# intel-aero/aero-optical-flow

Measured on AMD Instinct MI355X. Metric: frame-pairs/s (640x480, 8x8 SAD, +-4 search), higher is better.
Workload: dtype u8

## Files before the change

### aero-optical-flow_amd/csrc/aof_batch.cpp

```cpp
#include <cerrno>

#include "aof_ctx.hpp"

using namespace aof;

namespace {

struct Timed {
    aof_ctx *ctx; int id; hipStream_t s; bool on; int slot;
    Timed(aof_ctx *c, int k, hipStream_t st)
        : ctx(c), id(k), s(st), on(c->prof.on && !c->capturing && ((c->prof.mask >> k) & 1u)),
          slot((int)(c->prof.count[k] % AOF_PROFILE_RING))
    {
        if (on) (void)hipEventRecord(ctx->prof.ev[id][slot][0], s);
    }
    ~Timed() { if (on) { (void)hipEventRecord(ctx->prof.ev[id][slot][1], s); ctx->prof.count[id]++; } }
};

struct BatchView {
    const uint8_t *prev, *cur;
    int64_t stride;
    uint32_t *sums;
    uint8_t *l1_prev, *l1_cur;
    aof_block *blocks1; uint8_t *subdirs1; aof_flow *flows1; uint8_t *hist1;
    aof_block *blocks0; uint8_t *subdirs0; aof_flow *flows; uint8_t *hist0;
    uint32_t *hints;
};

enum SearchKind { SK_TILE16, SK_LANE8_GROUP, SK_LANE8, SK_GENERIC };
enum CoarseKind { COARSE_NONE, COARSE_FUSED, COARSE_K1 };

struct LevelPlan {
    SearchKind kind;
    bool refine;
    SearchArgs a;
    FlowTail tail;
};

struct BatchPlan {
    bool small;
    SmallArgs sm;
    CoarseKind coarse;
    bool k1_pass;
    bool sequence;
    CoarseArgs fused;
    PyramidArgs k1;
    LevelPlan level[2];
};

BatchView batch_view(const aof_ctx *ctx, const aof_ws_layout &L, const uint8_t *d_prev, const uint8_t *d_cur,
                     int64_t pair_stride, aof_block *d_blocks, uint8_t *d_subdirs, aof_flow *d_flows, void *d_workspace)
{
    const aof_params &p = ctx->params;
    BatchView v;
    uint8_t *ws = static_cast<uint8_t *>(d_workspace);
    const bool two = p.pyramid_levels == 2, eq = p.mean_subtract != 0;
    v.prev = d_prev; v.cur = d_cur; v.stride = pair_stride;
    v.sums = eq ? reinterpret_cast<uint32_t *>(ws + L.sums) : nullptr;
    v.l1_prev = two ? ws + L.l1_prev : nullptr;
    v.l1_cur = two ? ws + L.l1_cur : nullptr;
    v.blocks1 = reinterpret_cast<aof_block *>(ws + L.l1_blocks);
    v.subdirs1 = p.subpixel ? ws + L.l1_subdirs : nullptr;
    v.flows1 = reinterpret_cast<aof_flow *>(ws + L.l1_flows);
    v.hist1 = ws + L.l1_hist;
    v.blocks0 = d_blocks ? d_blocks : reinterpret_cast<aof_block *>(ws + L.l0_blocks);
    v.subdirs0 = nullptr;
    if (p.subpixel) v.subdirs0 = d_subdirs ? d_subdirs : ws + L.l0_subdirs;
    v.flows = d_flows;
    v.hist0 = ws + L.l0_hist;
    v.hints = p.tile == 16 ? reinterpret_cast<uint32_t *>(ws + L.hints) : nullptr;
    return v;
}

SearchArgs search_args(const aof_ctx *ctx, int level, const uint8_t *prev, const uint8_t *cur, int64_t stride,
                       aof_block *blocks, uint8_t *subdirs, const aof_flow *pred, const uint32_t *sums, int64_t n)
{
    const aof_params &p = ctx->params;
    SearchArgs a;
    a.prev = prev; a.cur = cur; a.pair_stride = stride;
    a.w = p.width >> level; a.h = p.height >> level;
    a.tile = p.tile; a.search = p.search;
    a.grid = level ? ctx->g1 : ctx->g0;
    a.feature_threshold = p.feature_threshold;
    a.value_threshold = value_threshold_u16(p);
    a.subpixel = p.subpixel;
    a.blocks = blocks; a.subdirs = p.subpixel ? subdirs : nullptr;
    a.pred = pred; a.sums = sums; a.level = level; a.n_pairs = n;
    a.hist_range = level_range(p, level);
    a.prune = ctx->search_mode;
    a.hints = nullptr;
    return a;
}

// ... 6 lines not shown
    if (a->prune && tile16_supported(x)) {
        a->prune = 0;
        return SK_TILE16;
    }
    if (lane8_supported(*a)) return lane8_group(*a) > 0 ? SK_LANE8_GROUP : SK_LANE8;
    return SK_GENERIC;
}

constexpr int64_t kSmallMaxPairs = 128;

FlowTail flow_tail(const aof_ctx *ctx, int level, aof_flow *flows, const aof_flow *pred)
{
    const aof_params &p = ctx->params;
    FlowTail t;
    t.nblocks = (level ? ctx->g1 : ctx->g0).blocks(); t.range = level_range(p, level);
    t.hist_filter = p.hist_filter; t.min_valid = p.min_valid;
    t.flows = flows; t.pred = pred; t.emit_predictor = level ? 1 : 0;
    return t;
}

LevelPlan plan_level(const aof_ctx *ctx, SearchArgs a, const FlowTail &tail)
{
    const SearchKind kind = search_kind(ctx, &a);
    return {kind, kind == SK_TILE16 && a.subpixel && !tile16_refines(a), a, tail};
}

BatchPlan plan_batch(const aof_ctx *ctx, const BatchView &v, int64_t n, bool k1_ready)
{
    const aof_params &p = ctx->params;
    const bool two = p.pyramid_levels == 2, eq = p.mean_subtract != 0;
    const int64_t frame = (int64_t)p.width * p.height, l1_frame = (int64_t)(p.width / 2) * (p.height / 2);
    BatchPlan P = {};
    const SmallArgs &sm = P.sm = {search_args(ctx, 0, v.prev, v.cur, v.stride, v.blocks0, v.subdirs0, nullptr, v.sums, n),
                                  search_args(ctx, 1, v.l1_prev, v.l1_cur, l1_frame, v.blocks1, v.subdirs1, nullptr, v.sums, n),
                                  flow_tail(ctx, 0, v.flows, two ? v.flows1 : nullptr), flow_tail(ctx, 1, v.flows1, nullptr),
                                  v.sums, two ? 2 : 1};
    SearchArgs a0 = sm.l0;
    a0.pred = sm.t0.pred;
    a0.hints = v.hints;
    P.level[0] = plan_level(ctx, a0, sm.t0);

    P.small = !ctx->force_generic && !ctx->split_coarse && n <= kSmallMaxPairs && P.level[0].kind == SK_LANE8_GROUP &&
              (!two || plan_level(ctx, sm.l1, sm.t1).kind == SK_LANE8_GROUP) && flow_small_supported(sm);
    if (P.small || (!two && !eq)) return P;

    CoarseArgs &c = P.fused;
    c.prev = v.prev; c.cur = v.cur; c.pair_stride = v.stride;
    c.w = p.width; c.h = p.height; c.tile = p.tile; c.search = p.search; c.subpixel = p.subpixel;
    c.grid = ctx->g1;
    c.feature_threshold = p.feature_threshold;
    c.value_threshold = value_threshold_u16(p);
    c.sums = v.sums; c.blocks = v.blocks1; c.tail = sm.t1; c.n_pairs = n;
    c.first_generation = ctx->cus; c.stagger_groups = 0; c.stagger_ticks = 0;
    if (two && !ctx->force_generic && !ctx->split_coarse && coarse_fused_supported(P.fused)) {
        P.coarse = COARSE_FUSED;
        return P;
    }
    P.coarse = COARSE_K1;
    const bool seq = P.sequence = v.cur - v.prev == frame && v.stride == frame && v.l1_cur >= v.l1_prev;
    P.k1 = {v.prev, seq ? nullptr : v.cur, v.stride, p.width, p.height, v.l1_prev, seq ? nullptr : v.l1_cur, v.sums,
            seq ? n + 1 : n, seq ? 1 : 0};
    P.k1_pass = !(P.sequence && k1_ready);
    if (two) {
// ... 24 lines not shown
        }
        if (arrived * 4 >= st.expected && seen) {
            st.stats.paying_pct = (int32_t)(paying * 100u / seen);
            st.belief = paying * 100u >= seen * kPayingPct ? 1 : 0;
            st.stats.belief = st.belief;
            st.stats.reports_read++;
        }
    }
    if (st.belief != 0) return true;
    if (++st.since_probe >= kProbeEvery) {
        st.since_probe = 0;
        return true;
    }
    return false;
}

enum Capture { CAPTURE_NONE, CAPTURE_ACTIVE, CAPTURE_UNKNOWN };

struct Lane8Launch {
    int prune;
    bool cols;
    bool fused;
    PruneReport rep;
};

VoteMem vote_mem(const aof_ctx *ctx) { return {ctx->votes.mem, kVoteStride, ctx->h_fault, ctx->votes.deadline_ticks}; }

Lane8Launch choose_lane8(aof_ctx *ctx, const SearchArgs &a, Capture cap)
{
    Lane8Launch l = {a.prune, false, false, {nullptr, 0, 1, 0}};
    if (l.prune && ctx->search_mode == AOF_SEARCH_ADAPTIVE) {
        AdaptiveSearch &st = ctx->adapt;
        if (!adaptive_lane8_prunes(st, a)) {
            l.prune = 0;
            st.stats.exhaustive_launches++;
        } else {
            l.prune = st.belief == 1 ? 1 : 2;
            if (++st.launch_no % 0x10000u == 0) st.launch_no++;
            l.rep.slots = st.slots;
            l.rep.launch_no = st.launch_no & 0xFFFFu;
            st.stats.pruned_launches++;
        }
    }
    SearchArgs x = a;
    x.prune = l.prune;
    l.cols = l.prune && lane8_cols_supported(x);
    const VoteMem vm = vote_mem(ctx);
    const bool fits = l.cols ? lane8_cols_votes_supported(x, vm, ctx->votes.pairs)
                             : (!l.prune && lane8_votes_supported(x, vm, ctx->votes.pairs));
    l.fused = fits && !ctx->votes.separate && (cap == CAPTURE_ACTIVE || (cap == CAPTURE_NONE && !ctx->votes.captured));
    return l;
}

int launch_lane8(aof_ctx *ctx, SearchArgs a, const FlowTail &tail, hipStream_t s, bool *reduced)
{
    hipStreamCaptureStatus status = hipStreamCaptureStatusNone;
    const Capture cap = hipStreamIsCapturing(s, &status) != hipSuccess ? CAPTURE_UNKNOWN
                        : status == hipStreamCaptureStatusNone         ? CAPTURE_NONE
                                                                       : CAPTURE_ACTIVE;
    Lane8Launch l = choose_lane8(ctx, a, cap);
    a.prune = l.prune;
    const bool eager = cap == CAPTURE_NONE;
    if (l.fused && eager && ctx->votes.used && ctx->votes.stream != s && hipStreamWaitEvent(s, ctx->votes.done, 0) != hipSuccess)
        return fail(ctx, -EIO, "cannot order the launch behind the context's previous one");
    const VoteMem vm = vote_mem(ctx);
    const FlowTail *t = l.fused ? &tail : nullptr;
    const VoteMem *m = l.fused ? &vm : nullptr;
    PruneReport *rep = l.prune ? &l.rep : nullptr;
    int rc = l.cols ? launch_search_lane8_cols(a, s, rep, t, m) : launch_search_lane8(a, s, t, m, rep);
    if (!rc && l.fused && eager) {
        rc = (int)hipEventRecord(ctx->votes.done, s);
        ctx->votes.stream = s;
        ctx->votes.used = true;
    } else if (!rc && l.fused) {
        ctx->votes.captured = true;
    }
    *reduced = l.fused;
    if (rep && l.rep.slots) ctx->adapt.expected = l.rep.expected;
    return rc;
}


int enqueue_level(aof_ctx *ctx, const LevelPlan &l, uint8_t *hist, int kid_search, int kid_reduce, hipStream_t s)
{
    bool reduced = l.kind == SK_LANE8_GROUP;
    {
        Timed t(ctx, kid_search, s);
        int rc;
        switch (l.kind) {
        case SK_TILE16:
            rc = launch_search_tile16(l.a, s);
            if (!rc && l.refine) rc = launch_refine(l.a, s);
            break;
        case SK_LANE8_GROUP:
            rc = launch_flow_lane8(l.a, l.tail, s);
            break;
        case SK_LANE8:
            rc = launch_lane8(ctx, l.a, l.tail, s, &reduced);
            if (rc < 0) return rc;
            break;
        default:
            rc = launch_search_generic(l.a, s);
        }
        if (rc) return fail(ctx, -EIO, "search launch: %s", hipGetErrorString((hipError_t)rc));
    }
    if (reduced) return 0;
    const ReduceArgs r = {l.a.blocks, l.a.subdirs, value_threshold_u16(ctx->params), l.tail, l.a.n_pairs, nullptr, 0,
                          reinterpret_cast<uint32_t *>(hist)};
    Timed t(ctx, kid_reduce, s);
    const int rc = launch_reduce(r, s);
    if (rc) return fail(ctx, -EIO, "reduce launch: %s", hipGetErrorString((hipError_t)rc));
    return 0;
}

int flow_batch(aof_ctx *ctx, const uint8_t *d_prev, const uint8_t *d_cur, int64_t pair_stride, int64_t n_pairs,
               aof_block *d_blocks, uint8_t *d_subdirs, aof_flow *d_flows, void *d_workspace, size_t workspace_bytes,
               void *stream, bool k1_ready)
{
    if (!ctx) return -EINVAL;
    if (n_pairs < 0 || (n_pairs > 0 && (!d_prev || !d_cur || !d_flows)))
        return fail(ctx, -EINVAL, "null frame or flow pointer");
    if (int sticky = sticky_error(ctx)) return sticky;
    if (n_pairs == 0) return 0;
    const aof_params &p = ctx->params;
    if (pair_stride < (int64_t)p.width * p.height && n_pairs > 1)
        return fail(ctx, -EINVAL, "pair_stride smaller than a frame");
    aof_ws_layout L;
    int rc = aof_workspace_layout(&p, n_pairs, &L);
    if (rc) return fail(ctx, rc, "bad workspace layout");
    if (!d_workspace || workspace_bytes < L.total_bytes)
        return fail(ctx, -ENOSPC, "workspace %zu B < required %zu B", workspace_bytes, L.total_bytes);
// ... 85 lines not shown
```

### aero-optical-flow_amd/csrc/aof_cols8_kernels.hpp

```cpp
#pragma once

#include <type_traits>

#include "aof_cols8_plan.hpp"
#include "aof_device.hpp"
#include "aof_internal.hpp"
#include "aof_lane8.hpp"
#include "aof_reduce.hpp"
#include "aof_refine.hpp"

namespace aof {

namespace {

template <bool SUBPIXEL, bool VOTE>
__device__ __forceinline__ void cols_walk(const SearchArgs &a, const ColsPlan &plan, const PruneReport &report, const VoteMem *votes)
{
    const uint32_t wg = blockIdx.x;
    const uint32_t unit0 = wg * blockDim.x + threadIdx.x;
    const bool in_tail = (uint32_t)__builtin_amdgcn_readfirstlane((int)unit0) >= plan.head_units;
    const ColsSegments sg = in_tail ? plan.tail : plan.head;
    const uint32_t unit = in_tail ? unit0 - plan.head_units : unit0;
    const uint32_t pair = (in_tail ? plan.head_pairs : 0u) + (uint32_t)__builtin_amdgcn_readfirstlane((int)fast_div(unit, sg.div_units));
    if (pair >= (uint32_t)a.n_pairs) return;
    const uint32_t local = unit - (pair - (in_tail ? plan.head_pairs : 0u)) * sg.units_per_pair;
    const uint32_t seg = fast_div(local, plan.div_nx), bx = local - __umul24(seg, (uint32_t)a.grid.nx);
    const bool live = local < (uint32_t)(sg.segs * a.grid.nx);
    const int by0 = (int)seg * sg.len;
    const int W = a.w;
    constexpr int m = SUBPIXEL ? 1 : 0;

    const uint64_t span = a.n_pairs > 1 ? (uint64_t)(a.n_pairs - pair) * (uint64_t)a.pair_stride : (uint64_t)a.w * (uint64_t)a.h;
    const uint32_t records = span > 0xFFFFFFFFull ? 0xFFFFFFFFu : (uint32_t)span;
    const int64_t base = (int64_t)pair * a.pair_stride;
    const __amdgpu_buffer_rsrc_t rs_prev = __builtin_amdgcn_make_buffer_rsrc(const_cast<uint8_t *>(a.prev) + base, 0, records, kRawBuffer);
    const __amdgpu_buffer_rsrc_t rs_cur = __builtin_amdgcn_make_buffer_rsrc(const_cast<uint8_t *>(a.cur) + base, 0, records, kRawBuffer);
    typedef const __attribute__((address_space(4))) uint32_t *const_u32;
    int px = 0, py = 0, delta = 0;
    if (a.pred) {
        const uint32_t w3 = ((const_u32)(a.pred + pair))[3];
// ... 31 lines not shown
    };
    uint4 win[16];
    {
        const int wy0 = a.grid.y0 + by0 * a.grid.step_y + py - 4;
        const uint32_t off_cur = (uint32_t)(__mul24(wy0, W) + wx0);
        if (mis != 0) {
            shifted_rows(off_cur, win);
        } else if (live) {
#pragma unroll
            for (int s = 0; s < 8; s++) {
                const u32x4 v = __builtin_amdgcn_raw_buffer_load_b128(rs_cur, off_cur, s * W, 0);
                win[s] = make_uint4(v.x, v.y, v.z, v.w);
            }
        }
        if (live && delta != 0) {
#pragma unroll
            for (int s = 0; s < 8; s++) win[s] = sat_add_u8x16(win[s], delta);
        }
    }
    int start_row = a.pred ? 4 : -1, prune_pays = a.prune == 2 ? 0 : 1;
    int seen = 0, paying = 0;
    std::conditional_t<VOTE && !SUBPIXEL, WalkVotes, NoWalkVotes> pending;
    pending.init();
    for (int step = 0; step < sg.len; step++) {
        const int by = by0 + step;
        const bool act = live && by < a.grid.ny;
        if (__ballot(act) == 0) break;
        const int j = a.grid.y0 + by * a.grid.step_y;
        const int wy0 = j + py - 4;
        const bool inside = act && column_inside && wy0 - m >= 0 && wy0 + 16 + m <= a.h;
        const uint32_t off_prev = (uint32_t)(__mul24(j, W) + i);
        const uint32_t off_cur8 = (uint32_t)(__mul24(wy0 + 8, W) + wx0);
        uint32_t ref[8][2];
        if (act) {
#pragma unroll
            for (int r = 0; r < 8; r++) {
                const u32x2 v = __builtin_amdgcn_raw_buffer_load_b64(rs_prev, off_prev, r * W, 2);
                ref[r][0] = v.x; ref[r][1] = v.y;
            }
            if (mis == 0) {
#pragma unroll
                for (int s = 8; s < 16; s++) {
                    const u32x4 v = __builtin_amdgcn_raw_buffer_load_b128(rs_cur, off_cur8, (s - 8) * W, 0);
                    win[s] = make_uint4(v.x, v.y, v.z, v.w);
                }
            }
// ... 46 lines not shown
                    if (!have_ring && rec.sad != 0) {
                        const uint32_t ring = off_cur8 + (uint32_t)((dyi - 9) * W + (dxi - 1));
                        uint32_t rows[10][3];
                        load_ring(rs_cur, ring, W, records, rows);
                        for_rows<-1, 8>([&](auto yc) {
                            constexpr int Y = decltype(yc)::value;
                            uint32_t d[3] = {rows[Y + 1][0], rows[Y + 1][1], rows[Y + 1][2]};
                            if (delta != 0) {
#pragma unroll
                                for (int q = 0; q < 3; q++) d[q] = sat_add_u8x4(d[q], delta);
                            }
                            st.template row<Y>(d, ref);
                        });
                    }
                    subdir = st.direction(rec.sad);
                }
            }
        }
        if (act) {
            const uint32_t slot = (uint32_t)(by * a.grid.nx) + bx;
            slots[slot] = __builtin_bit_cast(uint32_t, rec);
            if constexpr (SUBPIXEL) dirs[slot] = (uint8_t)subdir;
        }
        if constexpr (VOTE) {
            const bool ok = act && (uint32_t)rec.sad < (uint32_t)a.value_threshold;
            int hx = 0, hy = 0;
            if constexpr (SUBPIXEL) {
                hx = (subdir == 0 || subdir == 1 || subdir == 7) ? 1 : ((subdir == 3 || subdir == 4 || subdir == 5) ? -1 : 0);
                hy = (subdir == 1 || subdir == 2 || subdir == 3) ? 1 : ((subdir == 5 || subdir == 6 || subdir == 7) ? -1 : 0);
            }
            const int centre = 2 * a.hist_range + 1;
            if constexpr (SUBPIXEL) vote_and_arrive(*votes, a.hist_range, pair, act, ok, 2 * rec.dx + hx + centre, 2 * rec.dy + hy + centre);
            else pending.step(*votes, a.hist_range, pair, act, ok, 2 * rec.dx + hx + centre, 2 * rec.dy + hy + centre);
        }
#pragma unroll
        for (int s = 0; s < 8; s++) win[s] = win[s + 8];
    }
    if constexpr (VOTE) pending.flush(*votes, a.hist_range, pair);
    if (report.slots && threadIdx.x == 0 && wg % report.stride == 0)
        __hip_atomic_store(report.slots + wg / report.stride, (report.launch_no << 16) | ((uint32_t)paying << 8) | (uint32_t)seen,
                           __ATOMIC_RELAXED, __HIP_MEMORY_SCOPE_SYSTEM);
}

template <bool SUBPIXEL>
__global__ __launch_bounds__(kColsThreads, 4) void k_search_lane8_cols(SearchArgs a, ColsPlan plan, PruneReport report)
{
    cols_walk<SUBPIXEL, false>(a, plan, report, nullptr);
}

template <bool SUBPIXEL>
__global__ __launch_bounds__(kColsThreads, 4) void k_flow_lane8_cols(SearchArgs a, ColsPlan plan, PruneReport report, ColsVotes cv)
{
    if (blockIdx.x >= cv.search_wgs) {
        const uint32_t pair = (blockIdx.x - cv.search_wgs) * (blockDim.x >> 6) + (threadIdx.x >> 6);
        if (pair < (uint32_t)a.n_pairs) await_votes_and_finalise(cv.votes, cv.tail, pair);
        return;
    }
    cols_walk<SUBPIXEL, true>(a, plan, report, &cv.votes);
}

}

}
```

### aero-optical-flow_amd/csrc/aof_cols8_plan.hpp

```cpp
#pragma once

#include <cstdint>

#include "aof_internal.hpp"

namespace aof {

struct ColsSegments {
    int32_t segs, len;
    uint32_t units_per_pair;
    FastDiv div_units;
};
struct ColsPlan {
    ColsSegments head, tail;
    uint32_t head_pairs, head_units;
    FastDiv div_nx;
    uint32_t aligned;
};
struct ColsVotes {
    uint32_t search_wgs;
    FlowTail tail;
    VoteMem votes;
};


constexpr int kColsThreads = 256;
constexpr int kColsMaxRows = 8, kColsMinRows = 2;
constexpr int64_t kColsWavesWanted = 3072;
constexpr int64_t kWaveSlots = 4096;

}
```

### aero-optical-flow_amd/csrc/aof_internal.hpp

```cpp
#pragma once

#include <cstddef>
#include <cstdint>

#include "aof.h"

#if defined(__HIPCC__)
#define AOF_HD __host__ __device__
#else
#define AOF_HD
#endif

namespace aof {

struct FastDiv {
    uint32_t mul, shift;
};
inline FastDiv fastdiv_make(uint32_t d)
{
    FastDiv f = {0u, 0u};
    if (d == 0) return f;
    uint32_t l = 0;
    while ((1ull << l) < d) l++;
    f.mul = (uint32_t)(((1ull << 32) * ((1ull << l) - d)) / d + 1);
// ... 48 lines not shown
    int32_t value_threshold;
    int32_t subpixel;
    aof_block *blocks;
    uint8_t *subdirs;
    const aof_flow *pred;
    const uint32_t *sums;
    int32_t level;
    int64_t n_pairs;
    int32_t hist_range;
    int32_t prune;
    uint32_t *hints;
    FastDiv div_nb, div_nx;
};

struct ReduceArgs {
    const aof_block *blocks;
    const uint8_t *subdirs;
    int32_t value_threshold;
    FlowTail tail;
    int64_t n_pairs;
    const uint32_t *parts;
    int32_t nstrips;
    uint32_t *chunk_parts;
};

struct CoarseArgs {
    const uint8_t *prev, *cur;
    int64_t pair_stride;
    int32_t w, h;
    int32_t tile, search, subpixel;
    Grid grid;
    int32_t feature_threshold;
    int32_t value_threshold;
    uint32_t *sums;
    aof_block *blocks;
    FlowTail tail;
    int64_t n_pairs;
    FastDiv div_nb, div_nx, div_chunks;
    int32_t first_generation;
    int32_t stagger_groups, stagger_ticks;
    int32_t rows_per_sweep;
};

struct SmallArgs {
    SearchArgs l0, l1;
    FlowTail t0, t1;
// ... 4 lines not shown
struct PyramidArgs {
    const uint8_t *prev, *cur;
    int64_t pair_stride;
    int32_t w, h;
    uint8_t *l1_prev, *l1_cur;
    uint32_t *sums;
    int64_t n_pairs;
    int32_t sequence;
};

int launch_pyramid(const PyramidArgs &a, void *stream);
int launch_zero_words(uint32_t *words, int64_t count, void *stream);
bool coarse_fused_supported(const CoarseArgs &a);
int launch_coarse_fused(const CoarseArgs &a, void *stream);
int launch_search_generic(const SearchArgs &a, void *stream);
int launch_refine(const SearchArgs &a, void *stream);
bool lane8_supported(const SearchArgs &a);
bool lane8_votes_supported(const SearchArgs &a, const VoteMem &votes, int64_t capacity_pairs);
int launch_search_lane8(const SearchArgs &a, void *stream, const FlowTail *tail = nullptr,
                        const VoteMem *votes = nullptr, PruneReport *report = nullptr);
int64_t lane8_chunks(const SearchArgs &a);
bool lane8_cols_supported(const SearchArgs &a);
bool lane8_cols_votes_supported(const SearchArgs &a, const VoteMem &votes, int64_t capacity_pairs);
int launch_search_lane8_cols(const SearchArgs &a, void *stream, PruneReport *report = nullptr, const FlowTail *tail = nullptr,
                             const VoteMem *votes = nullptr);
constexpr int64_t kPruneMinChunks = 2048;
int lane8_group(const SearchArgs &a);
int launch_flow_lane8(const SearchArgs &a, const FlowTail &tail, void *stream);
bool tile16_supported(const SearchArgs &a);
bool tile16_refines(const SearchArgs &a);
int launch_search_tile16(const SearchArgs &a, void *stream);
bool flow_small_supported(const SmallArgs &a);
int launch_flow_small(const SmallArgs &a, void *stream);
int launch_flow_small_tagged(const SmallArgs &a, aof_flow *host_record, const uint32_t *tag, void *stream);
struct ResidentBox {
    unsigned long long word;
    uint32_t pad0[14];
    uint32_t done;
    uint32_t running;
    uint32_t exited;
    uint32_t started;
    uint32_t pad1[12];
};
static_assert(sizeof(ResidentBox) == 128, "two cache lines: host -> device, device -> host");
constexpr unsigned long long kResidentStopBit = 1ull << 63;
inline unsigned long long resident_word(uint32_t request, int slot, uint32_t prev_request)
{
    const unsigned long long prev = prev_request ? (unsigned long long)(prev_request & 0x3FFFFFFFu) + 1ull : 0ull;
// ... 49 lines not shown
```

### aero-optical-flow_amd/csrc/aof_lane8_launch.hpp

```cpp
#pragma once

#include <cstdint>

#include "aof_internal.hpp"

namespace aof {

struct ColsPlan;
struct ColsVotes;

int launch_k_search_lane8_ff(const SearchArgs &a, uint32_t items, uint32_t wgs, int threads, void *stream);
int launch_k_search_lane8_ft(const SearchArgs &a, uint32_t items, uint32_t wgs, int threads, void *stream);
int launch_k_search_lane8_tf(const SearchArgs &a, uint32_t items, uint32_t wgs, int threads, void *stream);
int launch_k_search_lane8_tt(const SearchArgs &a, uint32_t items, uint32_t wgs, int threads, void *stream);
int launch_k_flow_lane8_flat_ff(const SearchArgs &a, uint32_t items, uint32_t search_wgs, uint32_t grid, int threads, const FlowTail &t, const VoteMem &v, void *stream);
int launch_k_flow_lane8_flat_ft(const SearchArgs &a, uint32_t items, uint32_t search_wgs, uint32_t grid, int threads, const FlowTail &t, const VoteMem &v, void *stream);
int launch_k_flow_lane8_flat_tf(const SearchArgs &a, uint32_t items, uint32_t search_wgs, uint32_t grid, int threads, const FlowTail &t, const VoteMem &v, void *stream);
int launch_k_flow_lane8_flat_tt(const SearchArgs &a, uint32_t items, uint32_t search_wgs, uint32_t grid, int threads, const FlowTail &t, const VoteMem &v, void *stream);
int launch_k_search_lane8_pruned_f(const SearchArgs &a, uint32_t items, uint32_t wgs, int spw, const PruneReport &rep, void *stream);
int launch_k_search_lane8_pruned_t(const SearchArgs &a, uint32_t items, uint32_t wgs, int spw, const PruneReport &rep, void *stream);
int launch_k_flow_lane8_f(const SearchArgs &a, const FlowTail &t, int ppw, uint32_t wgs, size_t lds, void *stream);
int launch_k_flow_lane8_t(const SearchArgs &a, const FlowTail &t, int ppw, uint32_t wgs, size_t lds, void *stream);
int launch_k_search_lane8_cols_f(const SearchArgs &a, const ColsPlan &plan, const PruneReport &rep, uint32_t wgs, int threads, void *stream);
int launch_k_search_lane8_cols_t(const SearchArgs &a, const ColsPlan &plan, const PruneReport &rep, uint32_t wgs, int threads, void *stream);
int launch_k_flow_lane8_cols_f(const SearchArgs &a, const ColsPlan &plan, const PruneReport &rep, const ColsVotes &cv, uint32_t grid, int threads, void *stream);
int launch_k_flow_lane8_cols_t(const SearchArgs &a, const ColsPlan &plan, const PruneReport &rep, const ColsVotes &cv, uint32_t grid, int threads, void *stream);

}
```

### aero-optical-flow_amd/csrc/aof_reduce.hpp

```cpp
#pragma once

#include "aof_device.hpp"
#include "aof_internal.hpp"

namespace aof {

__device__ __forceinline__ void peak_window(int pos, int n, int *lo, int *hi)
{
    *lo = *hi = pos;
    if (pos > 1 && pos < n - 2) { *lo = pos - 2; *hi = pos + 2; }
    else if (pos == 0) { *hi = pos + 2; }
    else if (pos == n - 1) { *lo = pos - 2; }
    else if (pos == 1) { *lo = pos - 1; *hi = pos + 2; }
    else if (pos == n - 2) { *lo = pos - 2; *hi = pos + 1; }
}

template <typename T>
__device__ __forceinline__ T floor_div(T a, T b)
{
    T q = a / b;
    if ((a % b) < 0) q--;
    return q;
}

// ... 224 lines not shown
        const unsigned long long voters = __ballot(ok);
        const uint32_t nm = (uint32_t)__popcll(members), nv = (uint32_t)__popcll(voters);
        if (voters == 0) { arrivals = (uint32_t)__builtin_amdgcn_readfirstlane((int)(arrivals + nm)); return; }
        const int mine = bin_x | (bin_y << 8);
        const int k = __builtin_amdgcn_readlane(mine, __ffsll((long long)voters) - 1);
        if ((__ballot(ok && mine == k) & voters) == voters) {
            if (votes != 0 && key != k) flush(vm, range, pair);
            key = k;
            votes = (uint32_t)__builtin_amdgcn_readfirstlane((int)(votes + nv));
            arrivals = (uint32_t)__builtin_amdgcn_readfirstlane((int)(arrivals + nm));
            return;
        }
        flush(vm, range, pair);
        const int n = 2 * (2 * range + 1) + 1;
        uint32_t *rec = vm.base + (size_t)pair * vm.stride;
        wave_vote_agent(rec + 2, bin_x, ok);
        wave_vote_agent(rec + 2 + n, bin_y, ok);
        if ((threadIdx.x & 63) == 0)
            (void)__hip_atomic_fetch_add(reinterpret_cast<unsigned long long *>(rec), ((unsigned long long)nm << 32) | nv, __ATOMIC_RELAXED,
                                         __HIP_MEMORY_SCOPE_AGENT);
    }
};

__device__ __forceinline__ void await_votes_and_finalise(const VoteMem &vm, const FlowTail &tail, uint32_t pair)
{
    const uint64_t deadline_ticks = vm.deadline_ticks;
    const int centre = 2 * tail.range + 1, n = 2 * centre + 1, lane = (int)(threadIdx.x & 63);
    uint32_t *rec = vm.base + (size_t)pair * vm.stride, *hist_x = rec + 2, *hist_y = rec + 2 + n;
    const uint64_t t0 = __builtin_amdgcn_s_memrealtime();
    uint32_t hx = 0, hy = 0;
    int total = 0;
    bool complete = false;
    for (;;) {
        uint32_t arrived = 0, announced = 0;
        if (lane < n) {
            hx = __hip_atomic_load(&hist_x[lane], __ATOMIC_RELAXED, __HIP_MEMORY_SCOPE_AGENT);
            hy = __hip_atomic_load(&hist_y[lane], __ATOMIC_RELAXED, __HIP_MEMORY_SCOPE_AGENT);
        } else if (lane == 63) {
            const unsigned long long a = __hip_atomic_load(reinterpret_cast<unsigned long long *>(rec), __ATOMIC_RELAXED,
                                                           __HIP_MEMORY_SCOPE_AGENT);
            arrived = (uint32_t)(a >> 32);
            announced = (uint32_t)a;
        }
        arrived = (uint32_t)__shfl((int)arrived, 63, 64);
        announced = (uint32_t)__shfl((int)announced, 63, 64);
        total = (int)wave_sum_u32(hx);
// ... 47 lines not shown
```

### aero-optical-flow_amd/csrc/k_reduce.hip

```cpp
#include "aof_device.hpp"
#include "aof_internal.hpp"
#include "aof_reduce.hpp"

namespace aof {

namespace {

constexpr int kThreads = 256;
constexpr int kMaxHist = 256;
constexpr int64_t kMidPairs = 1024;
constexpr int64_t kWidePairs = 512;

template <int GROUP, int kThreads = 256>
__global__ __launch_bounds__(kThreads) void k_reduce(ReduceArgs a)
{
    constexpr int kGroups = kThreads / GROUP;
    __shared__ uint32_t s_hist[kGroups][2][kMaxHist];
    __shared__ int s_sums[kGroups][3];
    const int grp = (int)threadIdx.x / GROUP, tid = (int)threadIdx.x % GROUP;
    const int64_t pair = (int64_t)blockIdx.x * kGroups + grp;
    if (GROUP < kThreads && pair >= a.n_pairs) return;
    auto sync = [] { if (GROUP == kThreads) __syncthreads(); else __builtin_amdgcn_wave_barrier(); };
    uint32_t (*hist)[kMaxHist] = s_hist[grp];
    int *sums = s_sums[grp];
    const int centre = 2 * a.tail.range + 1, n = 2 * centre + 1;
    for (int k = tid; k < n; k += GROUP) { hist[0][k] = 0; hist[1][k] = 0; }
    if (tid < 3) sums[tid] = 0;
    sync();

    if (a.parts) {
        const uint32_t *parts = a.parts + (size_t)pair * a.nstrips * (size_t)(2 * n);
        for (int k = tid; k < 2 * n; k += GROUP) {
            uint32_t v = 0;
            for (int st = 0; st < a.nstrips; st++) v += parts[(size_t)st * (2 * n) + k];
            const int axis = k >= n, bin = k - axis * n;
            hist[axis][bin] = v;
            if (v) {
                atomicAdd(&sums[axis], (bin - centre) * (int)v);
                if (!axis) atomicAdd(&sums[2], (int)v);
            }
        }
        sync();
    } else {
    const aof_block *blocks = a.blocks + pair * a.tail.nblocks;
    const uint8_t *subdirs = a.subdirs ? a.subdirs + pair * a.tail.nblocks : nullptr;
    int s2x = 0, s2y = 0, cnt = 0;
    auto vote = [&](bool ok, aof_block r, int sd) {
        ok = ok && !(r.sad == AOF_SAD_SKIPPED || (int)r.sad >= a.value_threshold);
        int hx = 0, hy = 0;
        if (ok && subdirs) {
            hx = (sd == 0 || sd == 1 || sd == 7) ? 1 : ((sd == 3 || sd == 4 || sd == 5) ? -1 : 0);
            hy = (sd == 1 || sd == 2 || sd == 3) ? 1 : ((sd == 5 || sd == 6 || sd == 7) ? -1 : 0);
        }
// ... 98 lines not shown
        const bool in = b < b1;
        const aof_block r = __builtin_bit_cast(aof_block, in ? blocks[b] : 0xFFFF0000u);
        const int sd = in && subdirs ? subdirs[b] : 8;
        const bool ok = in && !(r.sad == AOF_SAD_SKIPPED || (int)r.sad >= a.value_threshold);
        int hx = 0, hy = 0;
        if (ok && subdirs) {
            hx = (sd == 0 || sd == 1 || sd == 7) ? 1 : ((sd == 3 || sd == 4 || sd == 5) ? -1 : 0);
            hy = (sd == 1 || sd == 2 || sd == 3) ? 1 : ((sd == 5 || sd == 6 || sd == 7) ? -1 : 0);
        }
        wave_vote(hist[0], 2 * r.dx + hx + centre, ok);
        wave_vote(hist[1], 2 * r.dy + hy + centre, ok);
    }
    __syncthreads();
    uint32_t *out = a.chunk_parts + ((size_t)pair * chunks + chunk) * (size_t)(2 * n);
    for (int k = tid; k < 2 * n; k += kThreads) out[k] = k < n ? hist[0][k] : hist[1][k - n];
}

}

int launch_reduce(const ReduceArgs &a, void *stream)
{
    if (a.n_pairs == 0) return 0;
    if (a.n_pairs > 0x7FFFFFFF) return (int)hipErrorInvalidValue;
    const int chunks = a.parts ? 0 : reduce_chunks(a.tail.nblocks);
    if (chunks > 0 && a.chunk_parts && a.n_pairs * chunks <= 0x7FFFFFFF) {
        hipLaunchKernelGGL(k_reduce_chunk, dim3((uint32_t)(a.n_pairs * chunks)), dim3(kThreads), 0,
                           static_cast<hipStream_t>(stream), a, chunks);
        ReduceArgs b = a;
        b.parts = a.chunk_parts;
        b.nstrips = chunks;
        hipLaunchKernelGGL(k_reduce<kThreads>, dim3((uint32_t)a.n_pairs), dim3(kThreads), 0,
                           static_cast<hipStream_t>(stream), b);
        return (int)hipGetLastError();
    }
    if (a.tail.nblocks <= 256 && !a.parts)
        hipLaunchKernelGGL(k_reduce<64>, dim3((uint32_t)((a.n_pairs + 3) / 4)), dim3(kThreads), 0,
                           static_cast<hipStream_t>(stream), a);
    else if (a.n_pairs <= kWidePairs && a.tail.nblocks >= 2048 && !a.parts)
        hipLaunchKernelGGL((k_reduce<1024, 1024>), dim3((uint32_t)a.n_pairs), dim3(1024), 0,
                           static_cast<hipStream_t>(stream), a);
    else if (a.n_pairs <= kMidPairs && a.tail.nblocks >= 2048 && !a.parts)
        hipLaunchKernelGGL((k_reduce<512, 512>), dim3((uint32_t)a.n_pairs), dim3(512), 0,
                           static_cast<hipStream_t>(stream), a);
    else
        hipLaunchKernelGGL(k_reduce<kThreads>, dim3((uint32_t)a.n_pairs), dim3(kThreads), 0,
                           static_cast<hipStream_t>(stream), a);
// ... 5 lines not shown
```

### aero-optical-flow_amd/csrc/k_search_cols8.hip

```cpp
#include <hip/hip_runtime.h>

#include "aof_cols8_plan.hpp"
#include "aof_internal.hpp"
#include "aof_lane8_launch.hpp"

namespace aof {

bool lane8_cols_supported(const SearchArgs &a)
{
    return lane8_supported(a) && a.grid.step_y == 8 && a.grid.nx >= 16 && a.grid.ny >= 2 && a.grid.blocks() > 256;
}

bool lane8_cols_votes_supported(const SearchArgs &a, const VoteMem &votes, int64_t capacity_pairs)
{
    const int n = 2 * (2 * a.hist_range + 1) + 1;
    if (!lane8_cols_supported(a) || !votes.base || !votes.fault || n > 62 || votes.stride < (uint32_t)(2 + 2 * n)) return false;
    return a.n_pairs <= capacity_pairs;
}

int launch_search_lane8_cols(const SearchArgs &a, void *stream, PruneReport *report, const FlowTail *tail, const VoteMem *votes)
{
    if (report) report->expected = 0;
    if (a.n_pairs == 0) return 0;
    if (!lane8_cols_supported(a) || (a.subpixel && !a.subdirs)) return (int)hipErrorInvalidValue;
    auto segments = [&](int len) {
        ColsSegments g;
        g.len = len > a.grid.ny ? a.grid.ny : len;
        g.segs = (a.grid.ny + g.len - 1) / g.len;
        g.units_per_pair = (uint32_t)((g.segs * a.grid.nx + 63) / 64 * 64);
        g.div_units = fastdiv_make(g.units_per_pair);
        return g;
    };
    auto waves = [&](int len) { return a.n_pairs * (int64_t)(segments(len).units_per_pair / 64); };
    int len = kColsMaxRows;
    while (len > kColsMinRows && waves(len) < kColsWavesWanted) len--;
    ColsPlan plan;
    plan.head = segments(len);
    plan.tail = segments(len / 2 < kColsMinRows ? kColsMinRows : len / 2);
    plan.div_nx = fastdiv_make((uint32_t)a.grid.nx);
    plan.aligned = (a.grid.step_x == 8 && a.w % 4 == 0 && a.pair_stride % 4 == 0 && reinterpret_cast<uintptr_t>(a.cur) % 4 == 0 &&
                    ((int64_t)a.w * a.h) % 4 == 0) ? 1u : 0u;
    const int64_t per = 0x7FFF0000ll / plan.tail.units_per_pair;
    for (int64_t done = 0; done < a.n_pairs; done += per) {
        SearchArgs s = a;
        s.n_pairs = a.n_pairs - done < per ? a.n_pairs - done : per;
        s.prev += done * a.pair_stride;
        s.cur += done * a.pair_stride;
        s.blocks += done * a.grid.blocks();
        if (s.subdirs) s.subdirs += done * a.grid.blocks();
        if (s.pred) s.pred += done;
        if (s.sums) s.sums += done * 4;
        const int64_t wpp = plan.head.units_per_pair / 64, all = s.n_pairs * wpp, rest = all % kWaveSlots;
        int64_t tail_pairs = 0;
        if (rest != 0 && rest * 5 < kWaveSlots * 4 && plan.tail.len < plan.head.len && all > kWaveSlots) tail_pairs = (rest + wpp - 1) / wpp;
        plan.head_pairs = (uint32_t)(s.n_pairs - tail_pairs);
        plan.head_units = plan.head_pairs * plan.head.units_per_pair;
        const int64_t units = (int64_t)plan.head_units + tail_pairs * plan.tail.units_per_pair;
        const int threads = kColsThreads;
        const int64_t wgs = (units + threads - 1) / threads;
        PruneReport rep = {nullptr, 0, 1, 0};
        if (report && report->slots && done == 0) {
            rep = *report;
            rep.stride = (uint32_t)((wgs + kPruneSlots - 1) / kPruneSlots);
            report->stride = rep.stride;
            report->expected = (uint32_t)((wgs + rep.stride - 1) / rep.stride);
        }
        int rc;
        if (tail && votes) {
            if (done != 0 || s.n_pairs != a.n_pairs) return (int)hipErrorInvalidValue;
            ColsVotes cv;
            cv.search_wgs = (uint32_t)wgs;
            cv.tail = *tail;
            cv.votes = *votes;
            const int64_t finalisers = (s.n_pairs + (threads >> 6) - 1) / (threads >> 6);
            rc = (s.subpixel ? launch_k_flow_lane8_cols_t : launch_k_flow_lane8_cols_f)(s, plan, rep, cv, (uint32_t)(wgs + finalisers), threads, stream);
        } else {
            rc = (s.subpixel ? launch_k_search_lane8_cols_t : launch_k_search_lane8_cols_f)(s, plan, rep, (uint32_t)wgs, threads, stream);
        }
        if (rc) return rc;
    }
    return 0;
}

}
```

Measured before the change: 7.938 million.

## Emit per-wave vote partials from cols search to shrink the reduce pass

```diff
diff --git a/aero-optical-flow_amd/csrc/aof_batch.cpp b/aero-optical-flow_amd/csrc/aof_batch.cpp
--- a/aero-optical-flow_amd/csrc/aof_batch.cpp
+++ b/aero-optical-flow_amd/csrc/aof_batch.cpp
@@ -25,6 +25,8 @@
     aof_block *blocks1; uint8_t *subdirs1; aof_flow *flows1; uint8_t *hist1;
     aof_block *blocks0; uint8_t *subdirs0; aof_flow *flows; uint8_t *hist0;
     uint32_t *hints;
+    uint8_t *l0_spare[2];
+    size_t l0_spare_per_pair[2];
 };
 
 enum SearchKind { SK_TILE16, SK_LANE8_GROUP, SK_LANE8, SK_GENERIC };
@@ -35,6 +37,7 @@
     bool refine;
     SearchArgs a;
     FlowTail tail;
+    uint32_t *parts;
 };
 
 struct BatchPlan {
@@ -69,6 +72,11 @@
     v.flows = d_flows;
     v.hist0 = ws + L.l0_hist;
     v.hints = p.tile == 16 ? reinterpret_cast<uint32_t *>(ws + L.hints) : nullptr;
+    const size_t nb0 = (size_t)ctx->g0.blocks();
+    v.l0_spare[0] = p.subpixel ? nullptr : ws + L.l0_subdirs;
+    v.l0_spare_per_pair[0] = nb0;
+    v.l0_spare[1] = d_blocks ? ws + L.l0_blocks : nullptr;
+    v.l0_spare_per_pair[1] = nb0 * sizeof(aof_block);
     return v;
 }
 
@@ -121,7 +129,30 @@
 LevelPlan plan_level(const aof_ctx *ctx, SearchArgs a, const FlowTail &tail)
 {
     const SearchKind kind = search_kind(ctx, &a);
-    return {kind, kind == SK_TILE16 && a.subpixel && !tile16_refines(a), a, tail};
+    return {kind, kind == SK_TILE16 && a.subpixel && !tile16_refines(a), a, tail, nullptr};
+}
+
+bool disjoint(const void *a, size_t a_bytes, const void *b, size_t b_bytes)
+{
+    const uintptr_t x = reinterpret_cast<uintptr_t>(a), y = reinterpret_cast<uintptr_t>(b);
+    return !a || !b || x + a_bytes <= y || y + b_bytes <= x;
+}
+
+uint32_t *wave_parts_room(const aof_ctx *ctx, const BatchView &v, const SearchArgs &a)
+{
+    const int rows = lane8_cols_part_rows(a);
+    if (rows == 0) return nullptr;
+    const size_t n = (size_t)a.n_pairs, nb = (size_t)a.grid.blocks(), bins = 2 * (2 * (size_t)a.hist_range + 1) + 1;
+    const size_t frames = (n - 1) * (size_t)v.stride + (size_t)ctx->params.width * (size_t)ctx->params.height;
+    for (int i = 0; i < 2; i++) {
+        uint8_t *r = v.l0_spare[i];
+        if (!r || (size_t)rows * bins * sizeof(uint32_t) > v.l0_spare_per_pair[i]) continue;
+        const size_t bytes = n * v.l0_spare_per_pair[i];
+        if (disjoint(r, bytes, a.prev, frames) && disjoint(r, bytes, a.cur, frames) && disjoint(r, bytes, a.blocks, n * nb * sizeof(aof_block)) &&
+            disjoint(r, bytes, a.subdirs, n * nb) && disjoint(r, bytes, v.flows, n * sizeof(aof_flow)))
+            return reinterpret_cast<uint32_t *>(r);
+    }
+    return nullptr;
 }
 
 BatchPlan plan_batch(const aof_ctx *ctx, const BatchView &v, int64_t n, bool k1_ready)
@@ -138,6 +169,7 @@
     a0.pred = sm.t0.pred;
     a0.hints = v.hints;
     P.level[0] = plan_level(ctx, a0, sm.t0);
+    if (P.level[0].kind == SK_LANE8) P.level[0].parts = wave_parts_room(ctx, v, a0);
 
     P.small = !ctx->force_generic && !ctx->split_coarse && n <= kSmallMaxPairs && P.level[0].kind == SK_LANE8_GROUP &&
               (!two || plan_level(ctx, sm.l1, sm.t1).kind == SK_LANE8_GROUP) && flow_small_supported(sm);
@@ -208,13 +240,15 @@
     bool cols;
     bool fused;
     PruneReport rep;
+    uint32_t *parts;
+    int part_rows;
 };
 
 VoteMem vote_mem(const aof_ctx *ctx) { return {ctx->votes.mem, kVoteStride, ctx->h_fault, ctx->votes.deadline_ticks}; }
 
-Lane8Launch choose_lane8(aof_ctx *ctx, const SearchArgs &a, Capture cap)
-{
-    Lane8Launch l = {a.prune, false, false, {nullptr, 0, 1, 0}};
+Lane8Launch choose_lane8(aof_ctx *ctx, const SearchArgs &a, Capture cap, uint32_t *room)
+{
+    Lane8Launch l = {a.prune, false, false, {nullptr, 0, 1, 0}, nullptr, 0};
     if (l.prune && ctx->search_mode == AOF_SEARCH_ADAPTIVE) {
         AdaptiveSearch &st = ctx->adapt;
         if (!adaptive_lane8_prunes(st, a)) {
@@ -235,16 +269,18 @@
     const bool fits = l.cols ? lane8_cols_votes_supported(x, vm, ctx->votes.pairs)
                              : (!l.prune && lane8_votes_supported(x, vm, ctx->votes.pairs));
     l.fused = fits && !ctx->votes.separate && (cap == CAPTURE_ACTIVE || (cap == CAPTURE_NONE && !ctx->votes.captured));
+    if (l.cols && !l.fused && room && (l.part_rows = lane8_cols_part_rows(x)) > 0) l.parts = room;
     return l;
 }
 
-int launch_lane8(aof_ctx *ctx, SearchArgs a, const FlowTail &tail, hipStream_t s, bool *reduced)
+int launch_lane8(aof_ctx *ctx, SearchArgs a, const FlowTail &tail, uint32_t *room, hipStream_t s, bool *reduced, uint32_t **parts,
+                 int *part_rows)
 {
     hipStreamCaptureStatus status = hipStreamCaptureStatusNone;
     const Capture cap = hipStreamIsCapturing(s, &status) != hipSuccess ? CAPTURE_UNKNOWN
                         : status == hipStreamCaptureStatusNone         ? CAPTURE_NONE
                                                                        : CAPTURE_ACTIVE;
-    Lane8Launch l = choose_lane8(ctx, a, cap);
+    Lane8Launch l = choose_lane8(ctx, a, cap, room);
     a.prune = l.prune;
     const bool eager = cap == CAPTURE_NONE;
     if (l.fused && eager && ctx->votes.used && ctx->votes.stream != s && hipStreamWaitEvent(s, ctx->votes.done, 0) != hipSuccess)
@@ -253,7 +289,7 @@
     const FlowTail *t = l.fused ? &tail : nullptr;
     const VoteMem *m = l.fused ? &vm : nullptr;
     PruneReport *rep = l.prune ? &l.rep : nullptr;
-    int rc = l.cols ? launch_search_lane8_cols(a, s, rep, t, m) : launch_search_lane8(a, s, t, m, rep);
+    int rc = l.cols ? launch_search_lane8_cols(a, s, rep, t, m, l.parts) : launch_search_lane8(a, s, t, m, rep);
     if (!rc && l.fused && eager) {
         rc = (int)hipEventRecord(ctx->votes.done, s);
         ctx->votes.stream = s;
@@ -262,6 +298,8 @@
         ctx->votes.captured = true;
     }
     *reduced = l.fused;
+    *parts = l.parts;
+    *part_rows = l.part_rows;
     if (rep && l.rep.slots) ctx->adapt.expected = l.rep.expected;
     return rc;
 }
@@ -270,6 +308,8 @@
 int enqueue_level(aof_ctx *ctx, const LevelPlan &l, uint8_t *hist, int kid_search, int kid_reduce, hipStream_t s)
 {
     bool reduced = l.kind == SK_LANE8_GROUP;
+    uint32_t *parts = nullptr;
+    int part_rows = 0;
     {
         Timed t(ctx, kid_search, s);
         int rc;
@@ -282,7 +322,7 @@
             rc = launch_flow_lane8(l.a, l.tail, s);
             break;
         case SK_LANE8:
-            rc = launch_lane8(ctx, l.a, l.tail, s, &reduced);
+            rc = launch_lane8(ctx, l.a, l.tail, l.parts, s, &reduced, &parts, &part_rows);
             if (rc < 0) return rc;
             break;
         default:
@@ -291,8 +331,8 @@
         if (rc) return fail(ctx, -EIO, "search launch: %s", hipGetErrorString((hipError_t)rc));
     }
     if (reduced) return 0;
-    const ReduceArgs r = {l.a.blocks, l.a.subdirs, value_threshold_u16(ctx->params), l.tail, l.a.n_pairs, nullptr, 0,
-                          reinterpret_cast<uint32_t *>(hist)};
+    const ReduceArgs r = {l.a.blocks, l.a.subdirs, value_threshold_u16(ctx->params), l.tail, l.a.n_pairs, nullptr, part_rows,
+                          reinterpret_cast<uint32_t *>(hist), parts};
     Timed t(ctx, kid_reduce, s);
     const int rc = launch_reduce(r, s);
     if (rc) return fail(ctx, -EIO, "reduce launch: %s", hipGetErrorString((hipError_t)rc));
diff --git a/aero-optical-flow_amd/csrc/aof_cols8_kernels.hpp b/aero-optical-flow_amd/csrc/aof_cols8_kernels.hpp
--- a/aero-optical-flow_amd/csrc/aof_cols8_kernels.hpp
+++ b/aero-optical-flow_amd/csrc/aof_cols8_kernels.hpp
@@ -13,9 +13,11 @@
 
 namespace {
 
-template <bool SUBPIXEL, bool VOTE>
-__device__ __forceinline__ void cols_walk(const SearchArgs &a, const ColsPlan &plan, const PruneReport &report, const VoteMem *votes)
-{
+template <bool SUBPIXEL, bool VOTE, bool PARTS = false>
+__device__ __forceinline__ void cols_walk(const SearchArgs &a, const ColsPlan &plan, const PruneReport &report, const VoteMem *votes,
+                                          const ColsParts &parts = {nullptr, 0}, uint32_t *lds = nullptr)
+{
+    static_assert(!(PARTS && (SUBPIXEL || VOTE)), "per-wave partials: integer votes of a walk without the in-launch reduction");
     const uint32_t wg = blockIdx.x;
     const uint32_t unit0 = wg * blockDim.x + threadIdx.x;
     const bool in_tail = (uint32_t)__builtin_amdgcn_readfirstlane((int)unit0) >= plan.head_units;
@@ -93,6 +95,9 @@
     int seen = 0, paying = 0;
     std::conditional_t<VOTE && !SUBPIXEL, WalkVotes, NoWalkVotes> pending;
     pending.init();
+    const int part_centre = 2 * a.hist_range + 1;
+    std::conditional_t<PARTS, WaveVotes, NoWaveVotes> parts_votes;
+    if constexpr (PARTS) parts_votes.init(lds, 2 * part_centre + 1);
     for (int step = 0; step < sg.len; step++) {
         const int by = by0 + step;
         const bool act = live && by < a.grid.ny;
@@ -185,6 +190,7 @@
             slots[slot] = __builtin_bit_cast(uint32_t, rec);
             if constexpr (SUBPIXEL) dirs[slot] = (uint8_t)subdir;
         }
+        if constexpr (PARTS) parts_votes.step(act && (uint32_t)rec.sad < (uint32_t)a.value_threshold, 2 * rec.dx + part_centre, 2 * rec.dy + part_centre);
         if constexpr (VOTE) {
             const bool ok = act && (uint32_t)rec.sad < (uint32_t)a.value_threshold;
             int hx = 0, hy = 0;
@@ -200,6 +206,11 @@
         for (int s = 0; s < 8; s++) win[s] = win[s + 8];
     }
     if constexpr (VOTE) pending.flush(*votes, a.hist_range, pair);
+    if constexpr (PARTS) {
+        const uint32_t rows = sg.units_per_pair >> 6, row = (uint32_t)__builtin_amdgcn_readfirstlane((int)local) >> 6;
+        const uint32_t zeros = row + rows < parts.rows ? (parts.rows - 1u - row) / rows : 0u;
+        parts_votes.store(parts.base + ((size_t)pair * parts.rows + row) * (uint32_t)(2 * part_centre + 1), (int)zeros, (int)rows);
+    }
     if (report.slots && threadIdx.x == 0 && wg % report.stride == 0)
         __hip_atomic_store(report.slots + wg / report.stride, (report.launch_no << 16) | ((uint32_t)paying << 8) | (uint32_t)seen,
                            __ATOMIC_RELAXED, __HIP_MEMORY_SCOPE_SYSTEM);
@@ -209,6 +220,14 @@
 __global__ __launch_bounds__(kColsThreads, 4) void k_search_lane8_cols(SearchArgs a, ColsPlan plan, PruneReport report)
 {
     cols_walk<SUBPIXEL, false>(a, plan, report, nullptr);
+}
+
+template <bool SUBPIXEL>
+__global__ __launch_bounds__(kColsThreads, 4) void k_search_lane8_cols_parts(SearchArgs a, ColsPlan plan, PruneReport report, ColsParts parts)
+{
+    static_assert(!SUBPIXEL, "partials: the integer walk only");
+    __shared__ uint32_t s_bins[kColsThreads / 64][2 * kPartsMaxBins];
+    cols_walk<SUBPIXEL, false, true>(a, plan, report, nullptr, parts, s_bins[threadIdx.x >> 6]);
 }
 
 template <bool SUBPIXEL>
diff --git a/aero-optical-flow_amd/csrc/aof_cols8_plan.hpp b/aero-optical-flow_amd/csrc/aof_cols8_plan.hpp
--- a/aero-optical-flow_amd/csrc/aof_cols8_plan.hpp
+++ b/aero-optical-flow_amd/csrc/aof_cols8_plan.hpp
@@ -22,11 +22,16 @@
     FlowTail tail;
     VoteMem votes;
 };
+struct ColsParts {
+    uint32_t *base;
+    uint32_t rows;
+};
 
 
 constexpr int kColsThreads = 256;
 constexpr int kColsMaxRows = 8, kColsMinRows = 2;
 constexpr int64_t kColsWavesWanted = 3072;
 constexpr int64_t kWaveSlots = 4096;
+constexpr int kPartsMaxBins = 64, kPartsMaxRows = 64;
 
 }
diff --git a/aero-optical-flow_amd/csrc/aof_internal.hpp b/aero-optical-flow_amd/csrc/aof_internal.hpp
--- a/aero-optical-flow_amd/csrc/aof_internal.hpp
+++ b/aero-optical-flow_amd/csrc/aof_internal.hpp
@@ -94,6 +94,7 @@
     const uint32_t *parts;
     int32_t nstrips;
     uint32_t *chunk_parts;
+    const uint32_t *wave_parts;
 };
 
 struct CoarseArgs {
@@ -144,8 +145,9 @@
 int64_t lane8_chunks(const SearchArgs &a);
 bool lane8_cols_supported(const SearchArgs &a);
 bool lane8_cols_votes_supported(const SearchArgs &a, const VoteMem &votes, int64_t capacity_pairs);
+int lane8_cols_part_rows(const SearchArgs &a);
 int launch_search_lane8_cols(const SearchArgs &a, void *stream, PruneReport *report = nullptr, const FlowTail *tail = nullptr,
-                             const VoteMem *votes = nullptr);
+                             const VoteMem *votes = nullptr, uint32_t *parts = nullptr);
 constexpr int64_t kPruneMinChunks = 2048;
 int lane8_group(const SearchArgs &a);
 int launch_flow_lane8(const SearchArgs &a, const FlowTail &tail, void *stream);
diff --git a/aero-optical-flow_amd/csrc/aof_lane8_launch.hpp b/aero-optical-flow_amd/csrc/aof_lane8_launch.hpp
--- a/aero-optical-flow_amd/csrc/aof_lane8_launch.hpp
+++ b/aero-optical-flow_amd/csrc/aof_lane8_launch.hpp
@@ -8,6 +8,7 @@
 
 struct ColsPlan;
 struct ColsVotes;
+struct ColsParts;
 
 int launch_k_search_lane8_ff(const SearchArgs &a, uint32_t items, uint32_t wgs, int threads, void *stream);
 int launch_k_search_lane8_ft(const SearchArgs &a, uint32_t items, uint32_t wgs, int threads, void *stream);
@@ -23,6 +24,7 @@
 int launch_k_flow_lane8_t(const SearchArgs &a, const FlowTail &t, int ppw, uint32_t wgs, size_t lds, void *stream);
 int launch_k_search_lane8_cols_f(const SearchArgs &a, const ColsPlan &plan, const PruneReport &rep, uint32_t wgs, int threads, void *stream);
 int launch_k_search_lane8_cols_t(const SearchArgs &a, const ColsPlan &plan, const PruneReport &rep, uint32_t wgs, int threads, void *stream);
+int launch_k_search_lane8_cols_parts_f(const SearchArgs &a, const ColsPlan &plan, const PruneReport &rep, const ColsParts &parts, uint32_t wgs, int threads, void *stream);
 int launch_k_flow_lane8_cols_f(const SearchArgs &a, const ColsPlan &plan, const PruneReport &rep, const ColsVotes &cv, uint32_t grid, int threads, void *stream);
 int launch_k_flow_lane8_cols_t(const SearchArgs &a, const ColsPlan &plan, const PruneReport &rep, const ColsVotes &cv, uint32_t grid, int threads, void *stream);
 
diff --git a/aero-optical-flow_amd/csrc/aof_reduce.hpp b/aero-optical-flow_amd/csrc/aof_reduce.hpp
--- a/aero-optical-flow_amd/csrc/aof_reduce.hpp
+++ b/aero-optical-flow_amd/csrc/aof_reduce.hpp
@@ -270,6 +270,62 @@
     }
 };
 
+struct NoWaveVotes {
+    __device__ __forceinline__ void init(uint32_t *, int) {}
+    __device__ __forceinline__ void step(bool, int, int) {}
+    __device__ __forceinline__ void store(uint32_t *, int, int) {}
+};
+struct WaveVotes {
+    uint32_t *bins;
+    int n, key;
+    uint32_t votes;
+
+    __device__ __forceinline__ void init(uint32_t *lds, int n_)
+    {
+        bins = lds; n = n_; key = 0; votes = 0;
+        const int lane = (int)(threadIdx.x & 63);
+        if (lane < n) { bins[2 * lane] = 0; bins[2 * lane + 1] = 0; }
+    }
+
+    __device__ __forceinline__ void flush()
+    {
+        if (votes == 0) return;
+        if ((threadIdx.x & 63) == 0) {
+            atomicAdd(&bins[key & 0xFF], votes);
+            atomicAdd(&bins[n + (key >> 8)], votes);
+        }
+        votes = 0;
+    }
+
+    __device__ __forceinline__ void step(bool ok, int bin_x, int bin_y)
+    {
+        const unsigned long long voters = __ballot(ok);
+        if (voters == 0) return;
+        const int mine = bin_x | (bin_y << 8);
+        const int k = __builtin_amdgcn_readlane(mine, __ffsll((long long)voters) - 1);
+        if ((__ballot(ok && mine == k) & voters) == voters) {
+            if (votes != 0 && key != k) flush();
+            key = k;
+            votes = (uint32_t)__builtin_amdgcn_readfirstlane((int)(votes + (uint32_t)__popcll(voters)));
+            return;
+        }
+        flush();
+        wave_vote(bins, bin_x, ok);
+        wave_vote(bins + n, bin_y, ok);
+    }
+
+    __device__ __forceinline__ void store(uint32_t *row, int zeros = 0, int gap = 0)
+    {
+        flush();
+        __builtin_amdgcn_wave_barrier();
+        const int lane = (int)(threadIdx.x & 63);
+        if (lane < n) {
+            row[lane] = bins[2 * lane] | (bins[2 * lane + 1] << 16);
+            for (int z = 1; z <= zeros; z++) row[(size_t)z * gap * n + lane] = 0u;
+        }
+    }
+};
+
 __device__ __forceinline__ void await_votes_and_finalise(const VoteMem &vm, const FlowTail &tail, uint32_t pair)
 {
     const uint64_t deadline_ticks = vm.deadline_ticks;
diff --git a/aero-optical-flow_amd/csrc/k_reduce.hip b/aero-optical-flow_amd/csrc/k_reduce.hip
--- a/aero-optical-flow_amd/csrc/k_reduce.hip
+++ b/aero-optical-flow_amd/csrc/k_reduce.hip
@@ -1,3 +1,4 @@
+#include "aof_cols8_plan.hpp"
 #include "aof_device.hpp"
 #include "aof_internal.hpp"
 #include "aof_reduce.hpp"
@@ -28,7 +29,31 @@
     if (tid < 3) sums[tid] = 0;
     sync();
 
-    if (a.parts) {
+    if (GROUP == 64 && a.wave_parts) {
+        constexpr int kRows = 32;
+        const uint32_t *rows = a.wave_parts + (size_t)pair * a.nstrips * (size_t)n;
+        for (int k = tid; k < n; k += GROUP) {
+            uint32_t lo = 0, hi = 0;
+            for (int st0 = 0; st0 < a.nstrips; st0 += kRows) {
+                uint32_t w[kRows];
+#pragma unroll
+                for (int st = 0; st < kRows; st++) w[st] = st0 + st < a.nstrips ? rows[(size_t)(st0 + st) * n + k] : 0u;
+#pragma unroll
+                for (int st = 0; st < kRows; st++) { lo += w[st] & 0xFFFFu; hi += w[st] >> 16; }
+            }
+#pragma unroll
+            for (int h = 0; h < 2; h++) {
+                const uint32_t v = h ? hi : lo;
+                const int b = 2 * k + h, axis = b >= n, bin = b - axis * n;
+                hist[axis][bin] = v;
+                if (v) {
+                    atomicAdd(&sums[axis], (bin - centre) * (int)v);
+                    if (!axis) atomicAdd(&sums[2], (int)v);
+                }
+            }
+        }
+        sync();
+    } else if (a.parts) {
         const uint32_t *parts = a.parts + (size_t)pair * a.nstrips * (size_t)(2 * n);
         for (int k = tid; k < 2 * n; k += GROUP) {
             uint32_t v = 0;
@@ -173,6 +198,12 @@
 {
     if (a.n_pairs == 0) return 0;
     if (a.n_pairs > 0x7FFFFFFF) return (int)hipErrorInvalidValue;
+    if (a.wave_parts) {
+        if (a.nstrips < 1 || a.nstrips > kPartsMaxRows || 2 * (2 * a.tail.range + 1) + 1 > kPartsMaxBins) return (int)hipErrorInvalidValue;
+        hipLaunchKernelGGL(k_reduce<64>, dim3((uint32_t)((a.n_pairs + 3) / 4)), dim3(kThreads), 0,
+                           static_cast<hipStream_t>(stream), a);
+        return (int)hipGetLastError();
+    }
     const int chunks = a.parts ? 0 : reduce_chunks(a.tail.nblocks);
     if (chunks > 0 && a.chunk_parts && a.n_pairs * chunks <= 0x7FFFFFFF) {
         hipLaunchKernelGGL(k_reduce_chunk, dim3((uint32_t)(a.n_pairs * chunks)), dim3(kThreads), 0,
diff --git a/aero-optical-flow_amd/csrc/k_search_cols8.hip b/aero-optical-flow_amd/csrc/k_search_cols8.hip
--- a/aero-optical-flow_amd/csrc/k_search_cols8.hip
+++ b/aero-optical-flow_amd/csrc/k_search_cols8.hip
@@ -18,25 +18,50 @@
     return a.n_pairs <= capacity_pairs;
 }
 
-int launch_search_lane8_cols(const SearchArgs &a, void *stream, PruneReport *report, const FlowTail *tail, const VoteMem *votes)
+namespace {
+
+ColsSegments segments(const SearchArgs &a, int len)
+{
+    ColsSegments g;
+    g.len = len > a.grid.ny ? a.grid.ny : len;
+    g.segs = (a.grid.ny + g.len - 1) / g.len;
+    g.units_per_pair = (uint32_t)((g.segs * a.grid.nx + 63) / 64 * 64);
+    g.div_units = fastdiv_make(g.units_per_pair);
+    return g;
+}
+
+void plan_segments(const SearchArgs &a, ColsPlan *plan)
+{
+    auto waves = [&](int len) { return a.n_pairs * (int64_t)(segments(a, len).units_per_pair / 64); };
+    int len = kColsMaxRows;
+    while (len > kColsMinRows && waves(len) < kColsWavesWanted) len--;
+    plan->head = segments(a, len);
+    plan->tail = segments(a, len / 2 < kColsMinRows ? kColsMinRows : len / 2);
+}
+
+}
+
+int lane8_cols_part_rows(const SearchArgs &a)
+{
+    const int n = 2 * (2 * a.hist_range + 1) + 1;
+    if (a.n_pairs < 1 || a.subpixel || n > kPartsMaxBins || !lane8_cols_supported(a)) return 0;
+    ColsPlan plan;
+    plan_segments(a, &plan);
+    const uint32_t head = plan.head.units_per_pair / 64, tail = plan.tail.units_per_pair / 64, rows = head > tail ? head : tail;
+    return rows > (uint32_t)kPartsMaxRows ? 0 : (int)rows;
+}
+
+int launch_search_lane8_cols(const SearchArgs &a, void *stream, PruneReport *report, const FlowTail *tail, const VoteMem *votes,
+                             uint32_t *parts)
 {
     if (report) report->expected = 0;
     if (a.n_pairs == 0) return 0;
     if (!lane8_cols_supported(a) || (a.subpixel && !a.subdirs)) return (int)hipErrorInvalidValue;
-    auto segments = [&](int len) {
-        ColsSegments g;
-        g.len = len > a.grid.ny ? a.grid.ny : len;
-        g.segs = (a.grid.ny + g.len - 1) / g.len;
-        g.units_per_pair = (uint32_t)((g.segs * a.grid.nx + 63) / 64 * 64);
-        g.div_units = fastdiv_make(g.units_per_pair);
-        return g;
-    };
-    auto waves = [&](int len) { return a.n_pairs * (int64_t)(segments(len).units_per_pair / 64); };
-    int len = kColsMaxRows;
-    while (len > kColsMinRows && waves(len) < kColsWavesWanted) len--;
+    const int part_rows = parts ? lane8_cols_part_rows(a) : 0;
+    if (parts && (part_rows == 0 || (tail && votes))) return (int)hipErrorInvalidValue;
+    const int bins = 2 * (2 * a.hist_range + 1) + 1;
     ColsPlan plan;
-    plan.head = segments(len);
-    plan.tail = segments(len / 2 < kColsMinRows ? kColsMinRows : len / 2);
+    plan_segments(a, &plan);
     plan.div_nx = fastdiv_make((uint32_t)a.grid.nx);
     plan.aligned = (a.grid.step_x == 8 && a.w % 4 == 0 && a.pair_stride % 4 == 0 && reinterpret_cast<uintptr_t>(a.cur) % 4 == 0 &&
                     ((int64_t)a.w * a.h) % 4 == 0) ? 1u : 0u;
@@ -50,6 +75,7 @@
         if (s.subdirs) s.subdirs += done * a.grid.blocks();
         if (s.pred) s.pred += done;
         if (s.sums) s.sums += done * 4;
+        const ColsParts cp = {parts ? parts + (size_t)done * (size_t)part_rows * (size_t)bins : nullptr, (uint32_t)part_rows};
         const int64_t wpp = plan.head.units_per_pair / 64, all = s.n_pairs * wpp, rest = all % kWaveSlots;
         int64_t tail_pairs = 0;
         if (rest != 0 && rest * 5 < kWaveSlots * 4 && plan.tail.len < plan.head.len && all > kWaveSlots) tail_pairs = (rest + wpp - 1) / wpp;
@@ -75,7 +101,8 @@
             const int64_t finalisers = (s.n_pairs + (threads >> 6) - 1) / (threads >> 6);
             rc = (s.subpixel ? launch_k_flow_lane8_cols_t : launch_k_flow_lane8_cols_f)(s, plan, rep, cv, (uint32_t)(wgs + finalisers), threads, stream);
         } else {
-            rc = (s.subpixel ? launch_k_search_lane8_cols_t : launch_k_search_lane8_cols_f)(s, plan, rep, (uint32_t)wgs, threads, stream);
+            rc = cp.base ? launch_k_search_lane8_cols_parts_f(s, plan, rep, cp, (uint32_t)wgs, threads, stream)
+                         : (s.subpixel ? launch_k_search_lane8_cols_t : launch_k_search_lane8_cols_f)(s, plan, rep, (uint32_t)wgs, threads, stream);
         }
         if (rc) return rc;
     }
diff --git a/aero-optical-flow_amd/csrc/k_search_cols8_parts.hip b/aero-optical-flow_amd/csrc/k_search_cols8_parts.hip
--- /dev/null
+++ b/aero-optical-flow_amd/csrc/k_search_cols8_parts.hip
@@ -0,0 +1,12 @@
+#include "aof_cols8_kernels.hpp"
+#include "aof_lane8_launch.hpp"
+
+namespace aof {
+
+int launch_k_search_lane8_cols_parts_f(const SearchArgs &a, const ColsPlan &plan, const PruneReport &rep, const ColsParts &parts, uint32_t wgs, int threads, void *stream)
+{
+    hipLaunchKernelGGL((k_search_lane8_cols_parts<false>), dim3(wgs), dim3(threads), 0, static_cast<hipStream_t>(stream), a, plan, rep, parts);
+    return (int)hipGetLastError();
+}
+
+}
```

Result: faster. 8.106 million (median of 6 runs) (+2.1%).
